# YooSungHyun/RNNTransducer

Measured on AMD Instinct MI355X. Metric: utterances/sec, higher is better.
Workload: dtype f32

## Files before the change

rnntransducer_amd/csrc/gemm_hp.hip:

```cpp
#include "common.hpp"

#include <stdlib.h>

namespace rnnt {
namespace {

typedef _Float16 f16x8 __attribute__((ext_vector_type(8)));
typedef __attribute__((address_space(3))) void lds_void;

constexpr int HP_BM = 256, HP_BN = 256, HP_BK = 32;
constexpr int HP_STAGE = (HP_BM + HP_BN) * 128;
constexpr int HP_RSRC = 0x00027000;

__device__ __forceinline__ float hp_scale_from_amax(unsigned amax_bits) {
  int eb = (int)((amax_bits >> 23) & 255u);
  if (eb == 0) return 1.0f;
  eb = eb < 15 ? 15 : eb;
  return __uint_as_float((unsigned)(268 - eb) << 23);
}
__device__ __forceinline__ float hp_inv_scale_from_amax(unsigned amax_bits) {
  int eb = (int)((amax_bits >> 23) & 255u);
  if (eb == 0) return 1.0f;
  eb = eb < 15 ? 15 : eb;
  return __uint_as_float((unsigned)(eb - 14) << 23);
}

__global__ void __launch_bounds__(256) hp_colmax_kernel(const float* __restrict__ x, long rows, int C, long ld, long rows_per_chunk,
                                                        unsigned* __restrict__ out) {
  const int c = blockIdx.x * 256 + threadIdx.x;
  if (c >= C) return;
  const long r0 = (long)blockIdx.y * rows_per_chunk, r1 = min(rows, r0 + rows_per_chunk);
  unsigned m = 0;
  for (long r = r0; r < r1; ++r) m = max(m, __float_as_uint(x[r * ld + c]) & 0x7fffffffu);
  if (m != 0) atomicMax(out + c, m);
}

__device__ __forceinline__ void hp_split8(const float (&x)[8], float scale, u32x4& hi, u32x4& lo) {
  f16x8 h, l;
#pragma unroll
  for (int e = 0; e < 8; ++e) {
    const float v = x[e] * scale;
    const _Float16 a = (_Float16)v;
    h[e] = a;
    l[e] = (_Float16)(v - (float)a);
  }
  hi = __builtin_bit_cast(u32x4, h);
  lo = __builtin_bit_cast(u32x4, l);
}

__global__ void __launch_bounds__(256) hp_split_kernel(const float* __restrict__ x, long rows, int K, long ld, unsigned* __restrict__ amax,
                                                       char* __restrict__ out, const int* __restrict__ rowidx) {
  const int Kp = (K + 31) & ~31, cpr = Kp >> 3;
  const int lane = threadIdx.x & 63;
  const bool vec = (ld & 3) == 0 && (reinterpret_cast<uintptr_t>(x) & 15) == 0;
  for (long ri = (long)blockIdx.x * 4 + (threadIdx.x >> 6); ri < rows; ri += (long)gridDim.x * 4) {
    const long r = rowidx ? (long)rowidx[ri] : ri;
    const float* row = x + r * ld;
    unsigned m = 0;
    for (int c = lane; c < cpr; c += 64) {
      const int k = 8 * c;
      if (vec && k + 7 < K) {
        const u32x4 a = *reinterpret_cast<const u32x4*>(row + k), b = *reinterpret_cast<const u32x4*>(row + k + 4);
#pragma unroll
        for (int e = 0; e < 4; ++e) m = max(m, max(a[e] & 0x7fffffffu, b[e] & 0x7fffffffu));
      } else {
#pragma unroll
        for (int e = 0; e < 8; ++e)
          if (k + e < K) m = max(m, __float_as_uint(row[k + e]) & 0x7fffffffu);
      }
    }
#pragma unroll
    for (int o = 32; o > 0; o >>= 1) m = max(m, (unsigned)__shfl_xor((int)m, o));
    if (lane == 0) amax[r] = m;
    const float scale = hp_scale_from_amax(m);
    for (int c = lane; c < cpr; c += 64) {
      const int k = 8 * c;
      float v[8];
      if (vec && k + 7 < K) {
        const f32x4 a = *reinterpret_cast<const f32x4*>(row + k), b = *reinterpret_cast<const f32x4*>(row + k + 4);
        v[0] = a[0]; v[1] = a[1]; v[2] = a[2]; v[3] = a[3]; v[4] = b[0]; v[5] = b[1]; v[6] = b[2]; v[7] = b[3];
      } else {
#pragma unroll
        for (int e = 0; e < 8; ++e) v[e] = (k + e < K) ? row[k + e] : 0.f;
      }
      u32x4 hi, lo;
      hp_split8(v, scale, hi, lo);
      char* dst = out + (r * (Kp >> 5) + (c >> 2)) * 128 + 16 * (c & 3);
      *reinterpret_cast<u32x4*>(dst) = hi;
      *reinterpret_cast<u32x4*>(dst + 64) = lo;
    }
  }
}

__global__ void __launch_bounds__(256) hp_split_t_kernel(const float* __restrict__ x, int R, int K, long ld, int Ksrc, int shift,
                                                         const unsigned* __restrict__ amax, char* __restrict__ out,
                                                         const int* __restrict__ kidx) {
  __shared__ float tile[32][257];
  const int kb = blockIdx.x, r0 = blockIdx.y * 256;
  const int tid = threadIdx.x;
  const bool vec = (ld & 3) == 0 && (reinterpret_cast<uintptr_t>(x) & 15) == 0;
#pragma unroll
  for (int q = 0; q < 8; ++q) {
    const int kk = 4 * q + (tid >> 6);
    const int kdst = kb * 32 + kk;
    const int ksrc = (kidx ? (kdst < K ? kidx[kdst] : 0) : kdst) + shift;
    const int c = 4 * (tid & 63);
    f32x4 v = {0.f, 0.f, 0.f, 0.f};
    if (kdst < K && ksrc >= 0 && ksrc < Ksrc) {
      const float* src = x + (long)ksrc * ld + r0 + c;
      if (vec && r0 + c + 3 < R) {
        v = *reinterpret_cast<const f32x4*>(src);
      } else {
#pragma unroll
        for (int e = 0; e < 4; ++e)
          if (r0 + c + e < R) v[e] = src[e];
      }
    }
#pragma unroll
    for (int e = 0; e < 4; ++e) tile[kk][c + e] = v[e];
  }
  __syncthreads();
  const int Kp32 = (K + 31) >> 5;
#pragma unroll
  for (int ps = 0; ps < 4; ++ps) {
    const int rl = (tid >> 2) + 64 * ps, ch = tid & 3;
    if (r0 + rl < R) {
      float v[8];
#pragma unroll
      for (int e = 0; e < 8; ++e) v[e] = tile[8 * ch + e][rl];
      u32x4 hi, lo;
      hp_split8(v, hp_scale_from_amax(amax[r0 + rl]), hi, lo);
      char* dst = out + ((long)(r0 + rl) * Kp32 + kb) * 128 + 16 * ch;
      *reinterpret_cast<u32x4*>(dst) = hi;
      *reinterpret_cast<u32x4*>(dst + 64) = lo;
    }
  }
}

__global__ void __launch_bounds__(256) hp_split_both_kernel(const float* __restrict__ x, int M, int C, long ld, const unsigned* __restrict__ rowmax,
                                                            const unsigned* __restrict__ colmax, char* __restrict__ out_rm, char* __restrict__ out_t,
                                                            const int* __restrict__ rowidx) {
  __shared__ float tile[32][257];
  const int kb = blockIdx.x, c0 = blockIdx.y * 256;
  const int tid = threadIdx.x;
  const int Cp = (C + 31) & ~31;
  const bool vec = (ld & 3) == 0 && (reinterpret_cast<uintptr_t>(x) & 15) == 0;
#pragma unroll
  for (int q = 0; q < 4; ++q) {
    const int row = 8 * q + (tid >> 5), col = 8 * (tid & 31);
    const int ri = kb * 32 + row, c = c0 + col;
    const int r = (rowidx && ri < M) ? rowidx[ri] : ri;
    float v[8] = {0.f, 0.f, 0.f, 0.f, 0.f, 0.f, 0.f, 0.f};
    if (ri < M && c < C) {
      const float* src = x + (long)r * ld + c;
      if (vec && c + 7 < C) {
        const f32x4 a = *reinterpret_cast<const f32x4*>(src), b = *reinterpret_cast<const f32x4*>(src + 4);
        v[0] = a[0]; v[1] = a[1]; v[2] = a[2]; v[3] = a[3]; v[4] = b[0]; v[5] = b[1]; v[6] = b[2]; v[7] = b[3];
      } else {
#pragma unroll
        for (int e = 0; e < 8; ++e)
          if (c + e < C) v[e] = src[e];
      }
    }
    if (ri < M && c < Cp) {
      u32x4 hi, lo;
      hp_split8(v, hp_scale_from_amax(rowmax[r]), hi, lo);
      char* dst = out_rm + ((long)r * (Cp >> 5) + (c >> 5)) * 128 + 16 * ((c >> 3) & 3);
      *reinterpret_cast<u32x4*>(dst) = hi;
      *reinterpret_cast<u32x4*>(dst + 64) = lo;
    }
#pragma unroll
    for (int e = 0; e < 8; ++e) tile[row][col + e] = v[e];
  }
  __syncthreads();
  const int Mp32 = (M + 31) >> 5;
#pragma unroll
  for (int ps = 0; ps < 4; ++ps) {
    const int rl = (tid >> 2) + 64 * ps, ch = tid & 3;
    if (c0 + rl < C) {
      float v[8];
#pragma unroll
      for (int e = 0; e < 8; ++e) v[e] = tile[8 * ch + e][rl];
      u32x4 hi, lo;
      hp_split8(v, hp_scale_from_amax(colmax[c0 + rl]), hi, lo);
      char* dst = out_t + ((long)(c0 + rl) * Mp32 + kb) * 128 + 16 * ch;
      *reinterpret_cast<u32x4*>(dst) = hi;
      *reinterpret_cast<u32x4*>(dst + 64) = lo;
    }
  }
}

struct HpGemmK {
  int M, N, nkt;
  const char* A; unsigned a_pitch, a_bytes;
  const char* B; unsigned b_pitch, b_bytes;
  const unsigned* a_amax; const unsigned* b_amax;
  float* C; int c_div; long c_so, c_si;
  const float* bias;
  unsigned flags;
  int splits, kt_per_split;
  float* slab;
  int tiles_m, tiles_n;
  int group_m;
  const int* a_rowidx;
  const int* c_rowidx;
};

__device__ __forceinline__ int hp_xcd_remap(int bid, int n) {
  const int q = n / 8, r = n % 8, xcd = bid % 8;
  return (xcd < r ? xcd * (q + 1) : r * (q + 1) + (xcd - r) * q) + bid / 8;
}

template <bool F16>
__device__ __forceinline__ void hp_tile256(const HpGemmK& p, const int bid, const int z, char* lds) {
  const int tid = threadIdx.x, lane = tid & 63;
  const int wave = __builtin_amdgcn_readfirstlane(tid >> 6);
  const int wr = wave >> 2, wc = wave & 3;
  const int m0 = (bid % p.tiles_m) * HP_BM, n0 = (bid / p.tiles_m) * HP_BN;

  const __amdgpu_buffer_rsrc_t ra = __builtin_amdgcn_make_buffer_rsrc(const_cast<char*>(p.A), 0, (int)p.a_bytes, HP_RSRC);
  const __amdgpu_buffer_rsrc_t rb = __builtin_amdgcn_make_buffer_rsrc(const_cast<char*>(p.B), 0, (int)p.b_bytes, HP_RSRC);

  unsigned va[4], vb[4];
  {
    const int src_slot = (lane & 7) ^ (((lane >> 4) & 3) | ((wave & 1) << 2));
#pragma unroll
    for (int j = 0; j < 4; ++j) {
      const int row = (8 * j + wave) * 8 + (lane >> 3);
      int ma = min(m0 + row, p.M - 1);
      const int nb = min(n0 + row, p.N - 1);
      if (p.a_rowidx) ma = p.a_rowidx[ma];
      va[j] = (unsigned)ma * p.a_pitch + 16u * src_slot;
      vb[j] = (unsigned)nb * p.b_pitch + 16u * src_slot;
    }
  }
  auto stage = [&](int buf, int kt) {
    char* base = lds + buf * HP_STAGE;
    const int koff = kt * 128;
#pragma unroll
    for (int j = 0; j < 4; ++j) {
      __builtin_amdgcn_raw_ptr_buffer_load_lds(ra, (lds_void*)(base + (8 * j + wave) * 1024), 16, va[j], koff, 0, 0);
      __builtin_amdgcn_raw_ptr_buffer_load_lds(rb, (lds_void*)(base + HP_BM * 128 + (8 * j + wave) * 1024), 16, vb[j], koff, 0, 0);
    }
  };

  const int frag0 = (lane & 15) * 128 + 16 * ((lane >> 4) ^ ((lane & 15) >> 1));
  const int a_base = wr * (128 * 128) + frag0;
  const int b_base = HP_BM * 128 + wc * (64 * 128) + frag0;

  f32x4 acc[8][4];
#pragma unroll
  for (int i = 0; i < 8; ++i)
#pragma unroll
    for (int j = 0; j < 4; ++j) acc[i][j] = (f32x4){0.f, 0.f, 0.f, 0.f};

  const int kt0 = z * p.kt_per_split;
  const int nk = min(p.nkt - kt0, p.kt_per_split);

  stage(0, kt0);
  asm volatile("s_waitcnt vmcnt(0)" ::: "memory");
  __syncthreads();
  for (int kt = 0; kt < nk; ++kt) {
    const int cur = kt & 1;
#ifndef HP_DBG_NO_DMA
    if (kt + 1 < nk) stage(cur ^ 1, kt0 + kt + 1);
#endif
    const char* sb = lds + cur * HP_STAGE;
    f16x8 a[4][2], b[2][2];
#ifdef HP_DBG_NO_LDSREAD
    auto load_a = [&](int mq) {
#pragma unroll
      for (int i = 0; i < 4; ++i) { asm volatile("" : "+v"(a[i][0]), "+v"(a[i][1])); }
    };
    auto load_b = [&](int nq) {
#pragma unroll
      for (int j = 0; j < 2; ++j) { asm volatile("" : "+v"(b[j][0]), "+v"(b[j][1])); }
    };
#else
    auto load_a = [&](int mq) {
#pragma unroll
      for (int i = 0; i < 4; ++i) {
        a[i][0] = *reinterpret_cast<const f16x8*>(sb + (a_base + (4 * mq + i) * 2048));
        if constexpr (!F16) a[i][1] = *reinterpret_cast<const f16x8*>(sb + ((a_base ^ 64) + (4 * mq + i) * 2048));
      }
    };
    auto load_b = [&](int nq) {
#pragma unroll
      for (int j = 0; j < 2; ++j) {
        b[j][0] = *reinterpret_cast<const f16x8*>(sb + (b_base + (2 * nq + j) * 2048));
        if constexpr (!F16) b[j][1] = *reinterpret_cast<const f16x8*>(sb + ((b_base ^ 64) + (2 * nq + j) * 2048));
      }
    };
#endif
    auto mma = [&](int mq, int nq) {
#pragma unroll
      for (int i = 0; i < 4; ++i)
#pragma unroll
        for (int j = 0; j < 2; ++j) {
          f32x4 c = acc[4 * mq + i][2 * nq + j];
          if constexpr (!F16) {
            c = __builtin_amdgcn_mfma_f32_16x16x32_f16(a[i][1], b[j][0], c, 0, 0, 0);
            c = __builtin_amdgcn_mfma_f32_16x16x32_f16(a[i][0], b[j][1], c, 0, 0, 0);
          }
          c = __builtin_amdgcn_mfma_f32_16x16x32_f16(a[i][0], b[j][0], c, 0, 0, 0);
          acc[4 * mq + i][2 * nq + j] = c;
        }
    };
#ifndef HP_DBG_NO_MFMA
    load_a(0); load_b(0); mma(0, 0);
    load_b(1); mma(0, 1);
    load_a(1); mma(1, 1);
    load_b(0); mma(1, 0);
#endif
    __builtin_amdgcn_sched_barrier(0);
#ifndef HP_DBG_NO_BARRIER
    __syncthreads();
#endif
  }
  const int mode = p.splits > 1 ? 0 : ((p.flags & RNNT_GEMM_ACCUM) ? 2 : 1);
  float* slab = p.splits > 1 ? p.slab + (long)z * p.M * p.N : nullptr;
  float bias_v[4], sb[4];
#pragma unroll
  for (int j = 0; j < 4; ++j) {
    const int n = n0 + wc * 64 + j * 16 + (lane & 15);
    bias_v[j] = (mode != 0 && p.bias && n < p.N) ? p.bias[n] : 0.f;
    sb[j] = hp_inv_scale_from_amax(p.b_amax[min(n, p.N - 1)]);
  }
#pragma unroll
  for (int i = 0; i < 8; ++i) {
#pragma unroll
    for (int reg = 0; reg < 4; ++reg) {
      const int m = m0 + wr * 128 + i * 16 + 4 * (lane >> 4) + reg;
      const bool mok = m < p.M;
      const int mc = mok ? m : 0;
      const float sa = hp_inv_scale_from_amax(p.a_amax[p.a_rowidx ? p.a_rowidx[mc] : mc]);
      const int mo = p.c_rowidx ? p.c_rowidx[mc] : mc;
      float* crow = mode == 0 ? slab + (long)mc * p.N : p.C + (long)(mo / p.c_div) * p.c_so + (long)(mo % p.c_div) * p.c_si;
      float old[4] = {0.f, 0.f, 0.f, 0.f};
      if (mode == 2) {
#pragma unroll
        for (int j = 0; j < 4; ++j) {
          const int n = n0 + wc * 64 + j * 16 + (lane & 15);
          if (mok && n < p.N) old[j] = crow[n];
        }
      }
#pragma unroll
      for (int j = 0; j < 4; ++j) {
        const int n = n0 + wc * 64 + j * 16 + (lane & 15);
        if (mok && n < p.N) crow[n] = acc[i][j][reg] * sa * sb[j] + bias_v[j] + old[j];
      }
    }
  }
}

__device__ __forceinline__ int hp_grouped_tile(int idx, int tiles_m, int tiles_n, int group_m) {
  const int band = group_m * tiles_n;
  const int g = idx / band, r = idx - g * band;
  const int m_first = g * group_m;
  const int gm = min(tiles_m - m_first, group_m);
  const int n = r / gm, m = m_first + (r - n * gm);
  return n * tiles_m + m;
}

template <bool F16>
__global__ void __launch_bounds__(512, 1) gemm_hp_kernel(const HpGemmK p) {
  extern __shared__ __attribute__((aligned(16))) char lds[];
  int bid = hp_xcd_remap(blockIdx.x, p.tiles_m * p.tiles_n);
  if (p.group_m > 0) bid = hp_grouped_tile(bid, p.tiles_m, p.tiles_n, p.group_m);
  hp_tile256<F16>(p, bid, blockIdx.y, lds);
}

constexpr int HPQ_MAX = 4;
struct HpGemmQ {
  HpGemmK prob[HPQ_MAX];
  int unit_end[HPQ_MAX];
  int nprob;
  unsigned xcd_skip;
  unsigned* counter;
};

template <bool F16>
__global__ void __launch_bounds__(512, 1) gemm_hpq_kernel(const HpGemmQ q) {
  extern __shared__ __attribute__((aligned(16))) char lds[];
  unsigned xcc;
  asm volatile("s_getreg_b32 %0, hwreg(HW_REG_XCC_ID)" : "=s"(xcc));
  xcc &= 7u;
  if ((q.xcd_skip >> xcc) & 1u) return;
  const unsigned allow = ~q.xcd_skip & 0xffu;
  const int nq = __builtin_popcount(allow);
  const int mine = __builtin_popcount(allow & ((1u << xcc) - 1u));
  int* next = reinterpret_cast<int*>(lds + 2 * HP_STAGE);
  const int total = q.unit_end[q.nprob - 1];
  for (int hop = 0; hop < nq; ++hop) {
    const int qi = (mine + hop) % nq;
    const int lo = (int)((long)total * qi / nq), hi = (int)((long)total * (qi + 1) / nq);
    while (true) {
      if (threadIdx.x == 0) {
        const int got = lo + (int)atomicAdd(q.counter + qi, 1u);
        *next = got;
        if (got < hi) atomicAdd(q.counter + 8, 1u);
      }
      __syncthreads();
      const int u = __builtin_amdgcn_readfirstlane(*next);
      __syncthreads();
      if (u >= hi) break;
      int pi = 0;
      while (u >= q.unit_end[pi]) ++pi;
      const HpGemmK& p = q.prob[pi];
      const int local = u - (pi ? q.unit_end[pi - 1] : 0);
      const int tn = local % p.tiles_n, z = (local / p.tiles_n) % p.splits, tm = local / (p.tiles_n * p.splits);
      hp_tile256<F16>(p, tn * p.tiles_m + tm, z, lds);
    }
  }
}

__global__ void hpq_check_kernel(unsigned* counter, unsigned total, unsigned* status) {
  if (counter[8] != total) {
    counter[9] = 1u;
    if (status) __hip_atomic_store(status, 2u, __ATOMIC_RELAXED, __HIP_MEMORY_SCOPE_AGENT);
  }
}

__global__ void __launch_bounds__(256) hp_splitk_reduce_kernel(const HpGemmK p) {
  const long total = (long)p.M * p.N;
  for (long i = (long)blockIdx.x * 256 + threadIdx.x; i < total; i += (long)gridDim.x * 256) {
    const int m = (int)(i / p.N), n = (int)(i % p.N);
    float s = 0.f;
    for (int z = 0; z < p.splits; ++z) s += p.slab[(long)z * total + i];
    if (p.bias) s += p.bias[n];
    const int mo = p.c_rowidx ? p.c_rowidx[m] : m;
    const long off = (long)(mo / p.c_div) * p.c_so + (long)(mo % p.c_div) * p.c_si + n;
    if (p.flags & RNNT_GEMM_ACCUM) s += p.C[off];
    p.C[off] = s;
  }
}

}

size_t hp_plane_bytes(int64_t rows, int64_t K) { return (size_t)rows * (size_t)ceil_div(K, 32) * 128; }

int hp_colmax(const float* x, int64_t rows, int64_t C, int64_t ld, uint32_t* amax, hipStream_t s) {
  RNNT_CHECK_HIP(hipMemsetAsync(amax, 0, (size_t)C * 4, s));
  if (rows == 0 || C == 0) return RNNT_OK;
  long chunks = ceil_div(2048, ceil_div(C, 256));
  if (chunks > ceil_div(rows, 64)) chunks = ceil_div(rows, 64);
  if (chunks < 1) chunks = 1;
  const long rpc = ceil_div(rows, chunks);
  ProfScope prof(RNNT_K_HP_SPLIT, 4.0 * (double)rows * (double)C, s);
  hipLaunchKernelGGL(hp_colmax_kernel, dim3((unsigned)ceil_div(C, 256), (unsigned)ceil_div(rows, rpc)), dim3(256), 0, s, x, (long)rows, (int)C,
                     (long)ld, rpc, amax);
  RNNT_CHECK_LAUNCH();
  return RNNT_OK;
}

int hp_split(const float* x, int64_t rows, int64_t K, int64_t ld, uint32_t* amax, void* planes, hipStream_t s, const int* rowidx) {
  if (rows == 0) return RNNT_OK;
  const long blocks = ceil_div(rows, 4);
  ProfScope prof(RNNT_K_HP_SPLIT, 8.0 * (double)rows * (double)K, s);
  hipLaunchKernelGGL(hp_split_kernel, dim3((unsigned)(blocks < 8192 ? blocks : 8192)), dim3(256), 0, s, x, (long)rows, (int)K, (long)ld, amax,
                     (char*)planes, rowidx);
  RNNT_CHECK_LAUNCH();
  return RNNT_OK;
}

int hp_split_t(const float* x, int64_t R, int64_t K, int64_t ld, int64_t Ksrc, int64_t shift, const uint32_t* amax, void* planes,
               hipStream_t s, const int* kidx) {
  if (R == 0 || K == 0) return RNNT_OK;
  ProfScope prof(RNNT_K_HP_SPLIT, 8.0 * (double)R * (double)K, s);
  hipLaunchKernelGGL(hp_split_t_kernel, dim3((unsigned)ceil_div(K, 32), (unsigned)ceil_div(R, 256)), dim3(256), 0, s, x, (int)R, (int)K, (long)ld,
                     (int)Ksrc, (int)shift, amax, (char*)planes, kidx);
  RNNT_CHECK_LAUNCH();
  return RNNT_OK;
}

int hp_split_both(const float* x, int64_t M, int64_t C, int64_t ld, const uint32_t* rowmax, const uint32_t* colmax, void* planes_rm,
                  void* planes_t, hipStream_t s, const int* rowidx) {
  if (M == 0 || C == 0) return RNNT_OK;
  ProfScope prof(RNNT_K_HP_SPLIT, 12.0 * (double)M * (double)C, s);
  hipLaunchKernelGGL(hp_split_both_kernel, dim3((unsigned)ceil_div(M, 32), (unsigned)ceil_div(C, 256)), dim3(256), 0, s, x, (int)M, (int)C, (long)ld,
                     rowmax, colmax, (char*)planes_rm, (char*)planes_t, rowidx);
  RNNT_CHECK_LAUNCH();
  return RNNT_OK;
}

struct HpGemmPlan {
  int tiles_m, tiles_n, group_m, splits, kt_per_split;
  size_t workspace_bytes_wanted;
};
static HpGemmPlan hp_gemm_plan(int64_t M, int64_t N, int64_t K, size_t workspace_bytes) {
  HpGemmPlan pl;
  pl.tiles_m = (int)ceil_div(M, HP_BM); pl.tiles_n = (int)ceil_div(N, HP_BN);
  const long tiles = (long)pl.tiles_m * pl.tiles_n;
  const long nkt = ceil_div(K, HP_BK);
  {
    static const int env_gm = getenv("RNNT_GEMM_HP_GROUP_M") ? atoi(getenv("RNNT_GEMM_HP_GROUP_M")) : -1;
    pl.group_m = env_gm >= 0 ? env_gm : (tiles >= 256 ? 8 : 4);
  }
  long want = 1;
  if (tiles < 192 && nkt >= 64) {
    want = ceil_div(256, tiles);
    if (want > nkt / 32) want = nkt / 32;
    if (want > 32) want = 32;
    if (want < 2) want = 1;
  }
  const size_t slab = (size_t)M * (size_t)N * 4;
  pl.workspace_bytes_wanted = want >= 2 ? (size_t)want * slab : 0;
  const size_t by_ws = workspace_bytes / slab;
  long splits = (size_t)want > by_ws ? (long)by_ws : want;
  if (splits < 2) splits = 1;
  pl.kt_per_split = (int)ceil_div(nkt, splits);
  pl.splits = (int)ceil_div(nkt, pl.kt_per_split);
  return pl;
}

size_t hp_gemm_workspace_bytes(int64_t M, int64_t N, int64_t K) { return hp_gemm_plan(M, N, K, 0).workspace_bytes_wanted; }

int hp_gemm(const void* A, const uint32_t* a_amax, const void* B, const uint32_t* b_amax, int64_t M, int64_t N, int64_t K, float* C,
            int64_t c_div, int64_t c_so, int64_t c_si, const float* bias, unsigned flags, void* workspace, size_t workspace_bytes,
            hipStream_t s, const int* a_rowidx, int64_t a_plane_rows, const int* c_rowidx) {
  RNNT_CHECK_ARG(A && B && C && a_amax && b_amax, "gemm_hp: null operand");
  RNNT_CHECK_ARG(!a_rowidx || a_plane_rows >= M, "gemm_hp: a gathered A operand needs the row count of its planes");
  RNNT_CHECK_ARG(M >= 1 && N >= 1 && K >= 1 && M < (1ll << 31) && N < (1ll << 31) && K < (1ll << 31), "gemm_hp: bad dims");
  RNNT_CHECK_ARG(c_div >= 1, "gemm_hp: c_div must be >= 1");
  RNNT_CHECK_ARG(((reinterpret_cast<uintptr_t>(A) | reinterpret_cast<uintptr_t>(B)) & 127) == 0, "gemm_hp: planes must be 128-byte aligned");
  HpGemmK k;
  k.M = (int)M; k.N = (int)N; k.nkt = (int)ceil_div(K, HP_BK);
  const size_t ab = hp_plane_bytes(a_rowidx ? a_plane_rows : M, K), bb = hp_plane_bytes(N, K);
  RNNT_CHECK_ARG(ab < (1ull << 32) && bb < (1ull << 32), "gemm_hp: an operand exceeds the 4 GB a buffer resource addresses");
  k.A = (const char*)A; k.a_pitch = (unsigned)k.nkt * 128u; k.a_bytes = (unsigned)ab;
  k.B = (const char*)B; k.b_pitch = (unsigned)k.nkt * 128u; k.b_bytes = (unsigned)bb;
  k.a_amax = a_amax; k.b_amax = b_amax;
  k.C = C; k.c_div = (int)(c_div > 0x7fffffff ? 0x7fffffff : c_div); k.c_so = c_so; k.c_si = c_si;
  k.bias = bias; k.flags = flags;
  k.a_rowidx = a_rowidx; k.c_rowidx = c_rowidx;
  const bool f16 = (flags & RNNT_GEMM_HP_F16) != 0u;
  const HpGemmPlan pl = hp_gemm_plan(M, N, K, workspace ? workspace_bytes : 0);
  k.tiles_m = pl.tiles_m; k.tiles_n = pl.tiles_n; k.group_m = pl.group_m;
  k.splits = pl.splits; k.kt_per_split = pl.kt_per_split;
  const int tiles = k.tiles_m * k.tiles_n, splits = k.splits;
  k.slab = (float*)workspace;
  if (f16) RNNT_CHECK_HIP(hipFuncSetAttribute((const void*)gemm_hp_kernel<true>, hipFuncAttributeMaxDynamicSharedMemorySize, 2 * HP_STAGE));
  else RNNT_CHECK_HIP(hipFuncSetAttribute((const void*)gemm_hp_kernel<false>, hipFuncAttributeMaxDynamicSharedMemorySize, 2 * HP_STAGE));
  {
    ProfScope prof(RNNT_K_GEMM_HP, 2.0 * (double)M * (double)N * (double)K, s);
    if (f16) hipLaunchKernelGGL(gemm_hp_kernel<true>, dim3(tiles, splits), dim3(512), 2 * HP_STAGE, s, k);
    else hipLaunchKernelGGL(gemm_hp_kernel<false>, dim3(tiles, splits), dim3(512), 2 * HP_STAGE, s, k);
    RNNT_CHECK_LAUNCH();
    if (splits > 1) {
      const long blocks = ceil_div((long)M * N, 256);
      hipLaunchKernelGGL(hp_splitk_reduce_kernel, dim3((unsigned)(blocks < 2048 ? blocks : 2048)), dim3(256), 0, s, k);
      RNNT_CHECK_LAUNCH();
    }
  }
  return RNNT_OK;
}

constexpr int HPQ_SPLIT_CAP = 8;
size_t hp_gemm_grouped_workspace_bytes(const int64_t* MN, int n) {
  size_t total = 0;
  for (int i = 0; i < n; ++i) total += align_up((size_t)HPQ_SPLIT_CAP * (size_t)MN[i] * 4, 256);
  return total;
}

int hp_gemm_grouped(const HpProblem* pr, int n, unsigned xcd_skip, unsigned* counter, void* workspace, size_t workspace_bytes,
                    hipStream_t s, unsigned* status) {
  RNNT_CHECK_ARG(pr && n >= 1 && n <= HPQ_MAX && counter, "gemm_hp grouped: 1..%d problems and a counter word", HPQ_MAX);
  RNNT_CHECK_ARG((xcd_skip & 0xffu) != 0xffu, "gemm_hp grouped: xcd_skip leaves no XCD");
  const bool f16 = (pr[0].flags & RNNT_GEMM_HP_F16) != 0u;
  for (int i = 1; i < n; ++i)
    RNNT_CHECK_ARG(((pr[i].flags & RNNT_GEMM_HP_F16) != 0u) == f16, "gemm_hp grouped: the problems of one launch share RNNT_GEMM_HP_F16");
  HpGemmQ q = {};
  q.nprob = n; q.xcd_skip = xcd_skip; q.counter = counter;
  int xcds = 0;
  for (int x = 0; x < 8; ++x) xcds += !((xcd_skip >> x) & 1u);
  const long workers = 32l * xcds;
  long total_kt = 0;
  double flops = 0.0;
  for (int i = 0; i < n; ++i) {
    const HpProblem& a = pr[i];
    RNNT_CHECK_ARG(a.A && a.B && a.C && a.a_amax && a.b_amax, "gemm_hp grouped: null operand (problem %d)", i);
    RNNT_CHECK_ARG(a.M >= 1 && a.N >= 1 && a.K >= 1 && a.M < (1ll << 31) && a.N < (1ll << 31) && a.K < (1ll << 31) && a.ldc >= a.N,
                   "gemm_hp grouped: bad dims (problem %d)", i);
    RNNT_CHECK_ARG(((reinterpret_cast<uintptr_t>(a.A) | reinterpret_cast<uintptr_t>(a.B)) & 127) == 0, "gemm_hp grouped: planes must be 128-byte aligned");
    HpGemmK& k = q.prob[i];
    k.M = (int)a.M; k.N = (int)a.N; k.nkt = (int)ceil_div(a.K, HP_BK);
    const size_t ab = hp_plane_bytes(a.M, a.K), bb = hp_plane_bytes(a.N, a.K);
    RNNT_CHECK_ARG(ab < (1ull << 32) && bb < (1ull << 32), "gemm_hp grouped: an operand exceeds the 4 GB a buffer resource addresses");
    k.A = (const char*)a.A; k.a_pitch = (unsigned)k.nkt * 128u; k.a_bytes = (unsigned)ab;
    k.B = (const char*)a.B; k.b_pitch = (unsigned)k.nkt * 128u; k.b_bytes = (unsigned)bb;
    k.a_amax = a.a_amax; k.b_amax = a.b_amax;
    k.C = a.C; k.c_div = 1; k.c_so = a.ldc; k.c_si = 0;
    k.bias = nullptr; k.flags = a.flags;
    k.a_rowidx = k.c_rowidx = nullptr;
    k.tiles_m = (int)ceil_div(a.M, HP_BM); k.tiles_n = (int)ceil_div(a.N, HP_BN);
    total_kt += (long)k.tiles_m * k.tiles_n * k.nkt;
    flops += 2.0 * (double)a.M * (double)a.N * (double)a.K;
  }
  long chunk = ceil_div(total_kt, 4 * workers);
  if (chunk < 32) chunk = 32;
  size_t off = 0;
  int units = 0;
  for (int i = 0; i < n; ++i) {
    HpGemmK& k = q.prob[i];
    long splits = ceil_div(k.nkt, chunk);
    if (splits > HPQ_SPLIT_CAP) splits = HPQ_SPLIT_CAP;
    const size_t per = (size_t)k.M * k.N * 4;
    while (splits > 1 && (!workspace || off + align_up((size_t)splits * per, 256) > workspace_bytes)) --splits;
    k.kt_per_split = (int)ceil_div(k.nkt, splits);
    k.splits = (int)ceil_div(k.nkt, k.kt_per_split);
    k.slab = k.splits > 1 ? reinterpret_cast<float*>((char*)workspace + off) : nullptr;
    if (k.splits > 1) off += align_up((size_t)k.splits * per, 256);
    units += k.tiles_m * k.tiles_n * k.splits;
    q.unit_end[i] = units;
  }
  RNNT_CHECK_HIP(hipMemsetAsync(counter, 0, 64, s));
  const int lds = 2 * HP_STAGE + 16;
  const void* qk = f16 ? (const void*)gemm_hpq_kernel<true> : (const void*)gemm_hpq_kernel<false>;
  RNNT_CHECK_HIP(hipFuncSetAttribute(qk, hipFuncAttributeMaxDynamicSharedMemorySize, lds));
  {
    ProfScope prof(RNNT_K_GEMM_HP, flops, s);
    int cus = 0, dev = 0;
    if (hipGetDevice(&dev) != hipSuccess || hipDeviceGetAttribute(&cus, hipDeviceAttributeMultiprocessorCount, dev) != hipSuccess || cus < 8) cus = 256;
    const dim3 grid(!xcd_skip && units < cus ? units : cus);
    if (f16) hipLaunchKernelGGL(gemm_hpq_kernel<true>, grid, dim3(512), lds, s, q);
    else hipLaunchKernelGGL(gemm_hpq_kernel<false>, grid, dim3(512), lds, s, q);
    RNNT_CHECK_LAUNCH();
    hipLaunchKernelGGL(hpq_check_kernel, dim3(1), dim3(1), 0, s, counter, (unsigned)units, status);
    RNNT_CHECK_LAUNCH();
    for (int i = 0; i < n; ++i)
      if (q.prob[i].splits > 1) {
        const long blocks = ceil_div((long)q.prob[i].M * q.prob[i].N, 256);
        hipLaunchKernelGGL(hp_splitk_reduce_kernel, dim3((unsigned)(blocks < 2048 ? blocks : 2048)), dim3(256), 0, s, q.prob[i]);
        RNNT_CHECK_LAUNCH();
      }
  }
  return RNNT_OK;
}

}

using namespace rnnt;

extern "C" size_t rnnt_hip_hp_bytes(int64_t rows, int64_t K) {
  if (rows < 0 || K < 0) return 0;
  return hp_plane_bytes(rows, K);
}

extern "C" int rnnt_hip_hp_split_ex(const float* x, int64_t rows, int64_t K, int64_t ld, int32_t transpose, int64_t src_rows, int64_t shift,
                                    void* planes, uint32_t* amax, int32_t amax_given, const int32_t* idx, void* stream) {
  RNNT_CHECK_ARG(x && planes && amax && rows >= 0 && K >= 0, "hp_split: bad arguments");
  RNNT_CHECK_ARG(rows < (1ll << 31) && K < (1ll << 31), "hp_split: dims must fit 31 bits");
  RNNT_CHECK_ARG((reinterpret_cast<uintptr_t>(planes) & 127) == 0, "hp_split: planes must be 128-byte aligned");
  hipStream_t s = (hipStream_t)stream;
  if (!transpose) {
    RNNT_CHECK_ARG(ld >= K, "hp_split: ld < K");
    RNNT_CHECK_ARG(!amax_given, "hp_split: the row-major split computes its row maxima itself");
    return hp_split(x, rows, K, ld, amax, planes, s, idx);
  }
  RNNT_CHECK_ARG(ld >= rows && src_rows >= 1, "hp_split: transposed source is (src_rows x >= rows), ld >= rows");
  RNNT_CHECK_ARG(src_rows < (1ll << 31) && shift > -(1ll << 31) && shift < (1ll << 31), "hp_split: src_rows and shift must fit 31 bits");
  if (!amax_given)
    if (int rc = hp_colmax(x, src_rows, rows, ld, amax, s)) return rc;
  return hp_split_t(x, rows, K, ld, src_rows, shift, amax, planes, s, idx);
}

extern "C" int rnnt_hip_hp_split(const float* x, int64_t rows, int64_t K, int64_t ld, int32_t transpose, int64_t src_rows, int64_t shift,
                                 void* planes, uint32_t* amax, int32_t amax_given, void* stream) {
  return rnnt_hip_hp_split_ex(x, rows, K, ld, transpose, src_rows, shift, planes, amax, amax_given, nullptr, stream);
}

extern "C" int rnnt_hip_hp_colmax(const float* x, int64_t rows, int64_t C, int64_t ld, uint32_t* amax, void* stream) {
  RNNT_CHECK_ARG(amax && rows >= 0 && C >= 0 && C < (1ll << 31), "hp_colmax: bad arguments");
  RNNT_CHECK_ARG(x || rows == 0 || C == 0, "hp_colmax: null source");
  RNNT_CHECK_ARG(ld >= C, "hp_colmax: ld < C");
  return hp_colmax(x, rows, C, ld, amax, (hipStream_t)stream);
}

extern "C" size_t rnnt_hip_gemm_hp_workspace_bytes(int64_t M, int64_t N, int64_t K) {
  if (M < 1 || N < 1 || K < 1) return 0;
  return hp_gemm_workspace_bytes(M, N, K);
}

extern "C" int rnnt_hip_gemm_hp_plan(int64_t M, int64_t N, int64_t K, size_t workspace_bytes, rnnt_hp_gemm_plan* out) {
  RNNT_CHECK_ARG(out != nullptr, "gemm_hp_plan: null plan");
  RNNT_CHECK_ARG(M >= 1 && N >= 1 && K >= 1 && M < (1ll << 31) && N < (1ll << 31) && K < (1ll << 31), "gemm_hp_plan: bad dims");
  const HpGemmPlan pl = hp_gemm_plan(M, N, K, workspace_bytes);
  out->tiles_m = pl.tiles_m; out->tiles_n = pl.tiles_n; out->group_m = pl.group_m;
  out->splits = pl.splits; out->kt_per_split = pl.kt_per_split;
  out->workspace_bytes_wanted = pl.workspace_bytes_wanted;
  return RNNT_OK;
}

extern "C" int rnnt_hip_gemm_hp_ex(const rnnt_hp_gemm_desc* d, void* stream) {
  RNNT_CHECK_ARG(d != nullptr, "gemm_hp: null descriptor");
  RNNT_CHECK_ARG(d->a_rowidx || d->a_plane_rows == 0, "gemm_hp: a_plane_rows given without a_rowidx");
  RNNT_CHECK_ARG(d->workspace || d->workspace_bytes == 0, "gemm_hp: workspace_bytes given without a workspace");
  return hp_gemm(d->A, d->a_amax, d->B, d->b_amax, d->M, d->N, d->K, d->C, d->c_div, d->c_so, d->c_si, d->bias, d->flags, d->workspace,
                 d->workspace_bytes, (hipStream_t)stream, d->a_rowidx, d->a_plane_rows, d->c_rowidx);
}

extern "C" int rnnt_hip_gemm_hp(const void* A, const uint32_t* a_amax, const void* B, const uint32_t* b_amax, int64_t M, int64_t N,
                                int64_t K, float* C, int64_t ldc, const float* bias, uint32_t flags, void* workspace,
                                size_t workspace_bytes, void* stream) {
  RNNT_CHECK_ARG(ldc >= N, "gemm_hp: ldc < N");
  return hp_gemm(A, a_amax, B, b_amax, M, N, K, C, 1, ldc, 0, bias, flags, workspace, workspace_bytes, (hipStream_t)stream);
}

static_assert(sizeof(rnnt_hp_problem) == sizeof(HpProblem), "rnnt_hp_problem mirrors HpProblem");

extern "C" size_t rnnt_hip_gemm_hp_grouped_workspace_bytes(const rnnt_hp_problem* problems, int32_t n) {
  if (!problems || n < 1 || n > HP_GROUP_MAX) return 0;
  int64_t mn[HP_GROUP_MAX];
  for (int i = 0; i < n; ++i) mn[i] = problems[i].M * problems[i].N;
  return 256 + hp_gemm_grouped_workspace_bytes(mn, n);
}

extern "C" int rnnt_hip_gemm_hp_grouped(const rnnt_hp_problem* problems, int32_t n, uint32_t xcd_skip, void* workspace,
                                        size_t workspace_bytes, void* stream) {
  RNNT_CHECK_ARG(problems && n >= 1 && n <= HP_GROUP_MAX, "gemm_hp grouped: 1..%d problems", HP_GROUP_MAX);
  RNNT_CHECK_ARG(workspace && workspace_bytes >= 256 && (reinterpret_cast<uintptr_t>(workspace) & 255) == 0,
                 "gemm_hp grouped: workspace of >= 256 bytes, 256-byte aligned");
  HpProblem pr[HP_GROUP_MAX];
  for (int i = 0; i < n; ++i) {
    const rnnt_hp_problem& a = problems[i];
    pr[i] = HpProblem{a.A, a.a_amax, a.B, a.b_amax, a.M, a.N, a.K, a.C, a.ldc, a.flags};
  }
  return hp_gemm_grouped(pr, n, xcd_skip, reinterpret_cast<unsigned*>(workspace), (char*)workspace + 256, workspace_bytes - 256,
                         (hipStream_t)stream);
}

extern "C" int rnnt_hip_hp_split_both_ex(const float* x, int64_t M, int64_t C, int64_t ld, const uint32_t* rowmax, const uint32_t* colmax,
                                         void* planes_rm, void* planes_t, const int32_t* rowidx, void* stream) {
  RNNT_CHECK_ARG(x && rowmax && colmax && planes_rm && planes_t && M >= 0 && C >= 0 && ld >= C, "hp_split_both: bad arguments");
  RNNT_CHECK_ARG(M < (1ll << 31) && C < (1ll << 31), "hp_split_both: dims must fit 31 bits");
  RNNT_CHECK_ARG(((reinterpret_cast<uintptr_t>(planes_rm) | reinterpret_cast<uintptr_t>(planes_t)) & 127) == 0, "hp_split_both: planes must be 128-byte aligned");
  return hp_split_both(x, M, C, ld, rowmax, colmax, planes_rm, planes_t, (hipStream_t)stream, rowidx);
}

extern "C" int rnnt_hip_hp_split_both(const float* x, int64_t M, int64_t C, int64_t ld, const uint32_t* rowmax, const uint32_t* colmax,
                                      void* planes_rm, void* planes_t, void* stream) {
  return rnnt_hip_hp_split_both_ex(x, M, C, ld, rowmax, colmax, planes_rm, planes_t, nullptr, stream);
}
```

Measured before the change: 1308.

## Pipeline HP GEMM k-loop with split-phase DMA and fine-grained vmcnt waits

Replaces the simple double-buffered k-loop with a two-tile-ahead pipeline. A and B tiles are staged in half-chunks interleaved between MFMA phases. Full-block syncs are replaced by per-phase barriers gated on specific vmcnt counts, and the next tile's A fragments are prefetched from the other LDS buffer. The B staging row mapping is permuted so each half-chunk covers the rows one compute phase consumes. This aims to hide global-to-LDS latency behind MFMA work, at the cost of more registers and fragile hand-tuned wait counts.

```diff
diff --git a/rnntransducer_amd/csrc/gemm_hp.hip b/rnntransducer_amd/csrc/gemm_hp.hip
--- a/rnntransducer_amd/csrc/gemm_hp.hip
+++ b/rnntransducer_amd/csrc/gemm_hp.hip
@@ -1,6 +1,8 @@
 #include "common.hpp"
 
 #include <stdlib.h>
+
+#include <type_traits>
 
 namespace rnnt {
 namespace {
@@ -222,26 +224,28 @@
   const __amdgpu_buffer_rsrc_t rb = __builtin_amdgcn_make_buffer_rsrc(const_cast<char*>(p.B), 0, (int)p.b_bytes, HP_RSRC);
 
   unsigned va[4], vb[4];
+  int blk_b[4];
   {
     const int src_slot = (lane & 7) ^ (((lane >> 4) & 3) | ((wave & 1) << 2));
 #pragma unroll
     for (int j = 0; j < 4; ++j) {
-      const int row = (8 * j + wave) * 8 + (lane >> 3);
-      int ma = min(m0 + row, p.M - 1);
-      const int nb = min(n0 + row, p.N - 1);
+      blk_b[j] = (wave & 3) | ((j & 1) << 2) | ((wave >> 2) << 3) | ((j >> 1) << 4);
+      int ma = min(m0 + (8 * j + wave) * 8 + (lane >> 3), p.M - 1);
+      const int nb = min(n0 + blk_b[j] * 8 + (lane >> 3), p.N - 1);
       if (p.a_rowidx) ma = p.a_rowidx[ma];
       va[j] = (unsigned)ma * p.a_pitch + 16u * src_slot;
       vb[j] = (unsigned)nb * p.b_pitch + 16u * src_slot;
     }
   }
-  auto stage = [&](int buf, int kt) {
-    char* base = lds + buf * HP_STAGE;
-    const int koff = kt * 128;
-#pragma unroll
-    for (int j = 0; j < 4; ++j) {
-      __builtin_amdgcn_raw_ptr_buffer_load_lds(ra, (lds_void*)(base + (8 * j + wave) * 1024), 16, va[j], koff, 0, 0);
-      __builtin_amdgcn_raw_ptr_buffer_load_lds(rb, (lds_void*)(base + HP_BM * 128 + (8 * j + wave) * 1024), 16, vb[j], koff, 0, 0);
-    }
+  auto stage_a = [&](int buf, int mq, int kt) {
+#pragma unroll
+    for (int j = mq; j < 4; j += 2)
+      __builtin_amdgcn_raw_ptr_buffer_load_lds(ra, (lds_void*)(lds + buf * HP_STAGE + (8 * j + wave) * 1024), 16, va[j], kt * 128, 0, 0);
+  };
+  auto stage_b = [&](int buf, int nq, int kt) {
+#pragma unroll
+    for (int j = nq; j < 4; j += 2)
+      __builtin_amdgcn_raw_ptr_buffer_load_lds(rb, (lds_void*)(lds + buf * HP_STAGE + HP_BM * 128 + blk_b[j] * 1024), 16, vb[j], kt * 128, 0, 0);
   };
 
   const int frag0 = (lane & 15) * 128 + 16 * ((lane >> 4) ^ ((lane & 15) >> 1));
@@ -257,38 +261,42 @@
   const int kt0 = z * p.kt_per_split;
   const int nk = min(p.nkt - kt0, p.kt_per_split);
 
-  stage(0, kt0);
-  asm volatile("s_waitcnt vmcnt(0)" ::: "memory");
-  __syncthreads();
-  for (int kt = 0; kt < nk; ++kt) {
-    const int cur = kt & 1;
-#ifndef HP_DBG_NO_DMA
-    if (kt + 1 < nk) stage(cur ^ 1, kt0 + kt + 1);
+#define HP_WAIT_VM(n) asm volatile("s_waitcnt vmcnt(" #n ")" ::: "memory")
+#define HP_WAIT_LDS() do { __builtin_amdgcn_s_waitcnt(0xC07F); asm volatile("" ::: "memory"); } while (0)
+#ifdef HP_DBG_NO_BARRIER
+#define HP_PHASE_SYNC(wait_vm) do { __builtin_amdgcn_sched_barrier(0); HP_WAIT_LDS(); \
+                                    __builtin_amdgcn_sched_barrier(0); } while (0)
+#else
+#define HP_PHASE_SYNC(wait_vm) do { __builtin_amdgcn_sched_barrier(0); wait_vm; HP_WAIT_LDS(); \
+                                    __builtin_amdgcn_s_barrier(); __builtin_amdgcn_sched_barrier(0); } while (0)
 #endif
-    const char* sb = lds + cur * HP_STAGE;
-    f16x8 a[4][2], b[2][2];
+  f16x8 a[2][4][2], b[2][2][2];
+  auto ktile = [&](auto cbuf, auto kind_c, const int kt) {
+    constexpr int C = decltype(cbuf)::value;
+    const int KIND = kind_c;
+    const char* sb = lds + C * HP_STAGE;
 #ifdef HP_DBG_NO_LDSREAD
-    auto load_a = [&](int mq) {
-#pragma unroll
-      for (int i = 0; i < 4; ++i) { asm volatile("" : "+v"(a[i][0]), "+v"(a[i][1])); }
+    auto load_a = [&](int mq, const char*) {
+#pragma unroll
+      for (int i = 0; i < 4; ++i) { asm volatile("" : "+v"(a[mq][i][0]), "+v"(a[mq][i][1])); }
     };
     auto load_b = [&](int nq) {
 #pragma unroll
-      for (int j = 0; j < 2; ++j) { asm volatile("" : "+v"(b[j][0]), "+v"(b[j][1])); }
+      for (int j = 0; j < 2; ++j) { asm volatile("" : "+v"(b[nq][j][0]), "+v"(b[nq][j][1])); }
     };
 #else
-    auto load_a = [&](int mq) {
+    auto load_a = [&](int mq, const char* st) {
 #pragma unroll
       for (int i = 0; i < 4; ++i) {
-        a[i][0] = *reinterpret_cast<const f16x8*>(sb + (a_base + (4 * mq + i) * 2048));
-        if constexpr (!F16) a[i][1] = *reinterpret_cast<const f16x8*>(sb + ((a_base ^ 64) + (4 * mq + i) * 2048));
+        a[mq][i][0] = *reinterpret_cast<const f16x8*>(st + (a_base + (4 * mq + i) * 2048));
+        if constexpr (!F16) a[mq][i][1] = *reinterpret_cast<const f16x8*>(st + ((a_base ^ 64) + (4 * mq + i) * 2048));
       }
     };
     auto load_b = [&](int nq) {
 #pragma unroll
       for (int j = 0; j < 2; ++j) {
-        b[j][0] = *reinterpret_cast<const f16x8*>(sb + (b_base + (2 * nq + j) * 2048));
-        if constexpr (!F16) b[j][1] = *reinterpret_cast<const f16x8*>(sb + ((b_base ^ 64) + (2 * nq + j) * 2048));
+        b[nq][j][0] = *reinterpret_cast<const f16x8*>(sb + (b_base + (2 * nq + j) * 2048));
+        if constexpr (!F16) b[nq][j][1] = *reinterpret_cast<const f16x8*>(sb + ((b_base ^ 64) + (2 * nq + j) * 2048));
       }
     };
 #endif
@@ -299,24 +307,81 @@
         for (int j = 0; j < 2; ++j) {
           f32x4 c = acc[4 * mq + i][2 * nq + j];
           if constexpr (!F16) {
-            c = __builtin_amdgcn_mfma_f32_16x16x32_f16(a[i][1], b[j][0], c, 0, 0, 0);
-            c = __builtin_amdgcn_mfma_f32_16x16x32_f16(a[i][0], b[j][1], c, 0, 0, 0);
+            c = __builtin_amdgcn_mfma_f32_16x16x32_f16(a[mq][i][1], b[nq][j][0], c, 0, 0, 0);
+            c = __builtin_amdgcn_mfma_f32_16x16x32_f16(a[mq][i][0], b[nq][j][1], c, 0, 0, 0);
           }
-          c = __builtin_amdgcn_mfma_f32_16x16x32_f16(a[i][0], b[j][0], c, 0, 0, 0);
+          c = __builtin_amdgcn_mfma_f32_16x16x32_f16(a[mq][i][0], b[nq][j][0], c, 0, 0, 0);
           acc[4 * mq + i][2 * nq + j] = c;
         }
     };
-#ifndef HP_DBG_NO_MFMA
-    load_a(0); load_b(0); mma(0, 0);
-    load_b(1); mma(0, 1);
-    load_a(1); mma(1, 1);
-    load_b(0); mma(1, 0);
+#if defined(HP_DBG_NO_DMA)
+    const bool FETCH = false;
+#else
+    const bool FETCH = KIND == 0;
 #endif
+#ifdef HP_DBG_NO_MFMA
+#define HP_COMPUTE(x) do { } while (0)
+#else
+#define HP_COMPUTE(x) do { x; } while (0)
+#endif
+    HP_COMPUTE(load_b(0));
+    if (KIND == 2) HP_PHASE_SYNC(HP_WAIT_VM(2)); else HP_PHASE_SYNC(HP_WAIT_VM(10));
+    HP_COMPUTE(load_b(1));
     __builtin_amdgcn_sched_barrier(0);
-#ifndef HP_DBG_NO_BARRIER
-    __syncthreads();
+    HP_COMPUTE(mma(0, 0));
+    __builtin_amdgcn_sched_barrier(0);
+    if (FETCH) { stage_a(C, 0, kt + 2); stage_b(C, 0, kt + 2); }
+    if (KIND == 0) HP_PHASE_SYNC(HP_WAIT_VM(12)); else if (KIND == 1) HP_PHASE_SYNC(HP_WAIT_VM(8)); else HP_PHASE_SYNC(HP_WAIT_VM(0));
+    HP_COMPUTE(load_a(1, sb));
+    __builtin_amdgcn_sched_barrier(0);
+    HP_COMPUTE(mma(0, 1));
+    __builtin_amdgcn_sched_barrier(0);
+    if (FETCH) stage_b(C, 1, kt + 2);
+    if (KIND == 0) HP_PHASE_SYNC(HP_WAIT_VM(10)); else if (KIND == 1) HP_PHASE_SYNC(HP_WAIT_VM(4)); else HP_PHASE_SYNC((void)0);
+    HP_COMPUTE(mma(1, 1));
+    __builtin_amdgcn_sched_barrier(0);
+    if (FETCH) stage_a(C, 1, kt + 2);
+    __builtin_amdgcn_sched_barrier(0);
+    if (KIND != 2) HP_COMPUTE(load_a(0, lds + (C ^ 1) * HP_STAGE));
+    __builtin_amdgcn_sched_barrier(0);
+    HP_COMPUTE(mma(1, 0));
+    __builtin_amdgcn_sched_barrier(0);
+  };
+  using std::integral_constant;
+  constexpr integral_constant<int, 0> c0{};
+  constexpr integral_constant<int, 1> c1{};
+
+  stage_a(0, 0, kt0); stage_b(0, 0, kt0); stage_b(0, 1, kt0); stage_a(0, 1, kt0);
+#ifndef HP_DBG_NO_DMA
+  if (nk > 1) {
+    stage_a(1, 0, kt0 + 1); stage_b(1, 0, kt0 + 1); stage_b(1, 1, kt0 + 1); stage_a(1, 1, kt0 + 1);
+    HP_WAIT_VM(12);
+  } else
 #endif
-  }
+  {
+    HP_WAIT_VM(4);
+  }
+  __builtin_amdgcn_s_barrier();
+#if !defined(HP_DBG_NO_MFMA) && !defined(HP_DBG_NO_LDSREAD)
+#pragma unroll
+  for (int i = 0; i < 4; ++i) {
+    a[0][i][0] = *reinterpret_cast<const f16x8*>(lds + (a_base + i * 2048));
+    if constexpr (!F16) a[0][i][1] = *reinterpret_cast<const f16x8*>(lds + ((a_base ^ 64) + i * 2048));
+  }
+#endif
+  int kt = 0;
+  for (; kt + 4 <= nk; kt += 2) {
+    ktile(c0, c0, kt0 + kt);
+    ktile(c1, c0, kt0 + kt + 1);
+  }
+  for (; kt < nk; kt += 2) {
+    ktile(c0, min(2, 3 - (nk - kt)), kt0 + kt);
+    if (kt + 1 < nk) ktile(c1, min(2, 4 - (nk - kt)), kt0 + kt + 1);
+  }
+#undef HP_COMPUTE
+#undef HP_PHASE_SYNC
+#undef HP_WAIT_LDS
+#undef HP_WAIT_VM
   const int mode = p.splits > 1 ? 0 : ((p.flags & RNNT_GEMM_ACCUM) ? 2 : 1);
   float* slab = p.splits > 1 ? p.slab + (long)z * p.M * p.N : nullptr;
   float bias_v[4], sb[4];
```

After: 1321 (median of 6 runs). Within noise of the previous version (+1.0%).

## Transpose MFMA operands and vectorize GEMM epilogue via LDS row/column tables

Applied to the files above, without the earlier changes.

Swaps the A/B operand order in the MFMA calls so each lane's accumulator holds four consecutive columns instead of four rows. This lets the epilogue write 16-byte vectors per row. Row offsets, A scales and validity flags, plus column scales and biases, are precomputed once per tile into LDS tables. A fast path for full, aligned tiles then does vectorized load/store with FMA. This targets scalar strided epilogue stores and the repeated per-element amax/rowidx lookups, at the cost of an extra block barrier and LDS reuse after the main loop.

```diff
diff --git a/rnntransducer_amd/csrc/gemm_hp.hip b/rnntransducer_amd/csrc/gemm_hp.hip
--- a/rnntransducer_amd/csrc/gemm_hp.hip
+++ b/rnntransducer_amd/csrc/gemm_hp.hip
@@ -1,6 +1,8 @@
 #include "common.hpp"
 
 #include <stdlib.h>
+
+#include <type_traits>
 
 namespace rnnt {
 namespace {
@@ -204,7 +206,14 @@
   int group_m;
   const int* a_rowidx;
   const int* c_rowidx;
+  int c_wide;
 };
+
+static void hp_set_c_wide(HpGemmK& k) {
+  const bool n4 = (k.N & 3) == 0;
+  if (k.splits > 1) k.c_wide = n4 && (reinterpret_cast<uintptr_t>(k.slab) & 15) == 0;
+  else k.c_wide = n4 && (reinterpret_cast<uintptr_t>(k.C) & 15) == 0 && (k.c_so & 3) == 0 && (k.c_si & 3) == 0;
+}
 
 __device__ __forceinline__ int hp_xcd_remap(int bid, int n) {
   const int q = n / 8, r = n % 8, xcd = bid % 8;
@@ -299,10 +308,10 @@
         for (int j = 0; j < 2; ++j) {
           f32x4 c = acc[4 * mq + i][2 * nq + j];
           if constexpr (!F16) {
-            c = __builtin_amdgcn_mfma_f32_16x16x32_f16(a[i][1], b[j][0], c, 0, 0, 0);
-            c = __builtin_amdgcn_mfma_f32_16x16x32_f16(a[i][0], b[j][1], c, 0, 0, 0);
+            c = __builtin_amdgcn_mfma_f32_16x16x32_f16(b[j][0], a[i][1], c, 0, 0, 0);
+            c = __builtin_amdgcn_mfma_f32_16x16x32_f16(b[j][1], a[i][0], c, 0, 0, 0);
           }
-          c = __builtin_amdgcn_mfma_f32_16x16x32_f16(a[i][0], b[j][0], c, 0, 0, 0);
+          c = __builtin_amdgcn_mfma_f32_16x16x32_f16(b[j][0], a[i][0], c, 0, 0, 0);
           acc[4 * mq + i][2 * nq + j] = c;
         }
     };
@@ -317,38 +326,78 @@
     __syncthreads();
 #endif
   }
+#ifdef HP_DBG_NO_BARRIER
+  __syncthreads();
+#endif
   const int mode = p.splits > 1 ? 0 : ((p.flags & RNNT_GEMM_ACCUM) ? 2 : 1);
-  float* slab = p.splits > 1 ? p.slab + (long)z * p.M * p.N : nullptr;
-  float bias_v[4], sb[4];
+  float* cbase = mode == 0 ? p.slab + (long)z * p.M * p.N : p.C;
+  u32x4* rtab = reinterpret_cast<u32x4*>(lds);
+  float* ctab_scale = reinterpret_cast<float*>(lds + 4096);
+  float* ctab_bias = reinterpret_cast<float*>(lds + 5120);
+  if (tid < 256) {
+    const int m = m0 + tid;
+    const bool mok = m < p.M;
+    const int mc = mok ? m : 0;
+    const float sa = hp_inv_scale_from_amax(p.a_amax[p.a_rowidx ? p.a_rowidx[mc] : mc]);
+    const int mo = p.c_rowidx ? p.c_rowidx[mc] : mc;
+    long off;
+    if (mode == 0) off = (long)mc * p.N;
+    else if (p.c_div == 1) off = (long)mo * p.c_so;
+    else off = (long)(mo / p.c_div) * p.c_so + (long)(mo % p.c_div) * p.c_si;
+    rtab[tid] = (u32x4){(unsigned)off, (unsigned)((unsigned long)off >> 32), __float_as_uint(sa), mok ? 1u : 0u};
+  } else {
+    const int t = tid - 256, n = n0 + t;
+    ctab_scale[t] = hp_inv_scale_from_amax(p.b_amax[min(n, p.N - 1)]);
+    ctab_bias[t] = (mode != 0 && p.bias && n < p.N) ? p.bias[n] : 0.f;
+  }
+  __syncthreads();
+  const int rl0 = wr * 128 + (lane & 15), cl0 = wc * 64 + 4 * (lane >> 4);
+  f32x4 sbv[4], bv[4];
 #pragma unroll
   for (int j = 0; j < 4; ++j) {
-    const int n = n0 + wc * 64 + j * 16 + (lane & 15);
-    bias_v[j] = (mode != 0 && p.bias && n < p.N) ? p.bias[n] : 0.f;
-    sb[j] = hp_inv_scale_from_amax(p.b_amax[min(n, p.N - 1)]);
-  }
-#pragma unroll
-  for (int i = 0; i < 8; ++i) {
-#pragma unroll
-    for (int reg = 0; reg < 4; ++reg) {
-      const int m = m0 + wr * 128 + i * 16 + 4 * (lane >> 4) + reg;
-      const bool mok = m < p.M;
-      const int mc = mok ? m : 0;
-      const float sa = hp_inv_scale_from_amax(p.a_amax[p.a_rowidx ? p.a_rowidx[mc] : mc]);
-      const int mo = p.c_rowidx ? p.c_rowidx[mc] : mc;
-      float* crow = mode == 0 ? slab + (long)mc * p.N : p.C + (long)(mo / p.c_div) * p.c_so + (long)(mo % p.c_div) * p.c_si;
-      float old[4] = {0.f, 0.f, 0.f, 0.f};
-      if (mode == 2) {
+    sbv[j] = *reinterpret_cast<const f32x4*>(ctab_scale + cl0 + 16 * j);
+    bv[j] = *reinterpret_cast<const f32x4*>(ctab_bias + cl0 + 16 * j);
+  }
+  if (p.c_wide && m0 + HP_BM <= p.M && n0 + HP_BN <= p.N) {
+    auto wide = [&](auto mode_c) {
+      constexpr int MODE = decltype(mode_c)::value;
+#pragma unroll
+      for (int i = 0; i < 8; ++i) {
+        const u32x4 e = rtab[rl0 + 16 * i];
+        const float sa = __uint_as_float(e[2]);
+        float* crow = cbase + (long)(((unsigned long)e[1] << 32) | e[0]) + (n0 + cl0);
+        f32x4 old[4];
+#pragma unroll
+        for (int j = 0; j < 4; ++j) old[j] = MODE == 2 ? *reinterpret_cast<const f32x4*>(crow + 16 * j) : (f32x4){0.f, 0.f, 0.f, 0.f};
 #pragma unroll
         for (int j = 0; j < 4; ++j) {
-          const int n = n0 + wc * 64 + j * 16 + (lane & 15);
-          if (mok && n < p.N) old[j] = crow[n];
+          f32x4 v;
+#pragma unroll
+          for (int r = 0; r < 4; ++r) v[r] = __builtin_fmaf(acc[i][j][r] * sa, sbv[j][r], bv[j][r]) + old[j][r];
+          *reinterpret_cast<f32x4*>(crow + 16 * j) = v;
         }
       }
-#pragma unroll
-      for (int j = 0; j < 4; ++j) {
-        const int n = n0 + wc * 64 + j * 16 + (lane & 15);
-        if (mok && n < p.N) crow[n] = acc[i][j][reg] * sa * sb[j] + bias_v[j] + old[j];
-      }
+    };
+    if (mode == 0) wide(std::integral_constant<int, 0>());
+    else if (mode == 1) wide(std::integral_constant<int, 1>());
+    else wide(std::integral_constant<int, 2>());
+  } else {
+#pragma unroll
+    for (int i = 0; i < 8; ++i) {
+      const u32x4 e = rtab[rl0 + 16 * i];
+      const float sa = __uint_as_float(e[2]);
+      const bool mok = e[3] != 0u;
+      float* crow = cbase + (long)(((unsigned long)e[1] << 32) | e[0]);
+#pragma unroll
+      for (int j = 0; j < 4; ++j)
+#pragma unroll
+        for (int r = 0; r < 4; ++r) {
+          const int n = n0 + cl0 + 16 * j + r;
+          if (mok && n < p.N) {
+            const float old = mode == 2 ? crow[n] : 0.f;
+            crow[n] = __builtin_fmaf(acc[i][j][r] * sa, sbv[j][r], bv[j][r]) + old;
+          }
+        }
     }
   }
 }
@@ -539,6 +588,7 @@
   k.splits = pl.splits; k.kt_per_split = pl.kt_per_split;
   const int tiles = k.tiles_m * k.tiles_n, splits = k.splits;
   k.slab = (float*)workspace;
+  hp_set_c_wide(k);
   if (f16) RNNT_CHECK_HIP(hipFuncSetAttribute((const void*)gemm_hp_kernel<true>, hipFuncAttributeMaxDynamicSharedMemorySize, 2 * HP_STAGE));
   else RNNT_CHECK_HIP(hipFuncSetAttribute((const void*)gemm_hp_kernel<false>, hipFuncAttributeMaxDynamicSharedMemorySize, 2 * HP_STAGE));
   {
@@ -610,6 +660,7 @@
     k.splits = (int)ceil_div(k.nkt, k.kt_per_split);
     k.slab = k.splits > 1 ? reinterpret_cast<float*>((char*)workspace + off) : nullptr;
     if (k.splits > 1) off += align_up((size_t)k.splits * per, 256);
+    hp_set_c_wide(k);
     units += k.tiles_m * k.tiles_n * k.splits;
     q.unit_end[i] = units;
   }
```

Result: no change. 1281 before, 1290 after (median of 6 runs) (+0.7%).
